# llrtt/G-NeRF

Measured on AMD Instinct MI355X. Metric: rays/sec at 128^2 neural render, 96 depth samples, higher is better.
Workload: dtype f32 (MLP products as compensated f16 hi/lo splits on MFMA, fp32 accumulate; exact-fp32 MFMA when the device-side range check says so)

## Files before the change

### g-nerf_amd/csrc/common.h

```cpp
#pragma once

#include <hip/hip_runtime.h>
#include <hip/hip_fp16.h>
#include <cstdarg>
#include <cstdio>
#include <cstdint>

#include "gnerf_hip.h"

namespace gnerf {

char* error_buffer();

inline int fail(int code, const char* fmt, ...) {
    va_list ap;
    va_start(ap, fmt);
    vsnprintf(error_buffer(), 512, fmt, ap);
    va_end(ap);
    return code;
}

inline int check_launch(const char* what) {
    hipError_t e = hipGetLastError();
    if (e != hipSuccess) return fail(GNERF_E_LAUNCH, "%s: %s", what, hipGetErrorString(e));
    return GNERF_OK;
}

inline hipStream_t as_stream(gnerf_stream_t s) { return reinterpret_cast<hipStream_t>(s); }

struct PerDeviceOnce {
    bool done[64] = {};
    template <class K> int raise_lds(K kernel, const char* what, int bytes = 160 * 1024) {
        int dev = 0;
        if (hipGetDevice(&dev) != hipSuccess || dev < 0 || dev >= 64) dev = -1;
        if (dev >= 0 && done[dev]) return GNERF_OK;
        if (hipFuncSetAttribute(reinterpret_cast<const void*>(kernel), hipFuncAttributeMaxDynamicSharedMemorySize, bytes) != hipSuccess)
            return fail(GNERF_E_LAUNCH, "%s: cannot raise the dynamic LDS limit", what);
        if (dev >= 0) done[dev] = true;
        return GNERF_OK;
    }
};

template <class T> struct Arith { typedef float type; };
template <> struct Arith<double> { typedef double type; };

template <class T> __device__ __forceinline__ typename Arith<T>::type load_as(const T* p, int64_t i) {
    return static_cast<typename Arith<T>::type>(p[i]);
}
template <> __device__ __forceinline__ float load_as<__half>(const __half* p, int64_t i) { return __half2float(p[i]); }

template <class T> __device__ __forceinline__ void store_as(T* p, int64_t i, typename Arith<T>::type v) { p[i] = static_cast<T>(v); }
template <> __device__ __forceinline__ void store_as<__half>(__half* p, int64_t i, float v) { p[i] = __float2half(v); }

constexpr int kNumCU = 256;
constexpr int kNumXCD = 8;

template <class T, int VEC> struct alignas(sizeof(T) * VEC) Pk { T v[VEC]; };
template <class T> __device__ __forceinline__ float round_to(float v) { return v; }
template <> __device__ __forceinline__ float round_to<__half>(float v) { return __half2float(__float2half(v)); }

constexpr int kActLrelu01 = 13;
template <class T, int VEC, int ACT, bool SCALE, bool NOISE, bool NEXT>
__device__ __forceinline__ Pk<T, VEC> modconv_epilogue_vec(const Pk<T, VEC>& in, const float (&sc)[VEC], float nz, bool round_noise, const float (&bv)[VEC],
                                                          const float (&nx)[VEC], float alpha, float gain, float clamp) {
    float t[VEC];
    if constexpr (sizeof(T) == 2 && VEC % 2 == 0 && (SCALE || NOISE)) {
        typedef _Float16 h2 __attribute__((ext_vector_type(2)));
#pragma unroll
        for (int k = 0; k < VEC; k += 2) {
            const h2 xv = {__builtin_bit_cast(_Float16, in.v[k]), __builtin_bit_cast(_Float16, in.v[k + 1])};
            const h2 s2 = {(_Float16)sc[k], (_Float16)sc[k + 1]};
            h2 r;
            if constexpr (NOISE) {
                if (round_noise || SCALE) {
                    const h2 n2 = {(_Float16)nz, (_Float16)nz};
                    r = __builtin_elementwise_fma(xv, s2, n2);
                } else {
                    r = (h2){(_Float16)((float)xv[0] + nz), (_Float16)((float)xv[1] + nz)};
                }
            } else {
                r = xv * s2;
            }
            t[k] = (float)r[0];
            t[k + 1] = (float)r[1];
        }
    } else {
#pragma unroll
        for (int k = 0; k < VEC; k++) {
            float uu = float(load_as<T>(in.v, k));
            if constexpr (SCALE || NOISE) uu = round_to<T>(fmaf(uu, SCALE ? round_to<T>(sc[k]) : 1.f, NOISE ? ((round_noise || SCALE) ? round_to<T>(nz) : nz) : 0.f));
            t[k] = uu;
        }
    }
    Pk<T, VEC> out;
    const bool slope01 = alpha >= 0.f && alpha <= 1.f;
#pragma unroll
    for (int k = 0; k < VEC; k++) {
        const float uu = t[k] + bv[k];
        float r = uu;
        if (ACT == 3) r = slope01 ? fmaxf(uu, uu * alpha) : (uu > 0.f ? uu : uu * alpha);
        if (ACT == kActLrelu01) r = fmaxf(uu, uu * alpha);
        r *= gain;
        if (clamp >= 0.f) r = __builtin_amdgcn_fmed3f(r, -clamp, clamp);
        if constexpr (sizeof(T) == 2 && VEC % 2 == 0) {
            t[k] = r;
        } else {
            if constexpr (NEXT) r = round_to<T>(r) * nx[k];
            store_as<T>(out.v, k, r);
// ... 18 lines not shown
```

### g-nerf_amd/csrc/planes.hip

```cpp

#include "common.h"
#include "raygen.h"

namespace {

using namespace gnerf;

#ifndef GNERF_REPACK_PX
#define GNERF_REPACK_PX 64
#endif
constexpr int CT = 32, PT = GNERF_REPACK_PX;

__device__ __forceinline__ unsigned abs_bits(float v) { return __float_as_uint(v) & 0x7fffffffu; }
__device__ __forceinline__ void publish_absmax(unsigned m, unsigned* out) {
    __shared__ unsigned wave_max[4];
#pragma unroll
    for (int o = 32; o > 0; o >>= 1) m = max(m, (unsigned)__shfl_xor((int)m, o));
    if ((threadIdx.x & 63) == 0) wave_max[threadIdx.x >> 6] = m;
    __syncthreads();
    if (threadIdx.x == 0) {
        const unsigned b = max(max(wave_max[0], wave_max[1]), max(wave_max[2], wave_max[3]));
        if (b > __hip_atomic_load(out, __ATOMIC_RELAXED, __HIP_MEMORY_SCOPE_AGENT)) atomicMax(out, b);
    }
}

template <bool STATS>
__global__ __launch_bounds__(256) void nchw_to_nhwc_kernel(const float* __restrict__ src, float* __restrict__ dst,
                                                           int c, int64_t hw, int tiles_p, int tiles_c, unsigned* absmax) {
    __shared__ float tile[CT][PT + 1];
    int64_t t = blockIdx.x;
    const int tp = int(t % tiles_p); t /= tiles_p;
    const int tc = int(t % tiles_c); t /= tiles_c;
    const int64_t plane = t;
    const int64_t p0 = int64_t(tp) * PT;
    const int c0 = tc * CT;
    const float* s = src + plane * c * hw;
    float* d = dst + plane * hw * c;
    unsigned amax = 0u;
#pragma unroll
    for (int i = 0; i < CT * PT / 256; i++) {
        const int e = threadIdx.x + 256 * i;
        const int ch = e / PT, px = e % PT;
        float v = 0.f;
        if (c0 + ch < c && p0 + px < hw) v = s[int64_t(c0 + ch) * hw + p0 + px];
        tile[ch][px] = v;
        if (STATS) amax = max(amax, abs_bits(v));
    }
    __syncthreads();
#pragma unroll
    for (int i = 0; i < CT * PT / 256; i++) {
        const int e = threadIdx.x + 256 * i;
        const int px = e / CT, ch = e % CT;
        if (c0 + ch < c && p0 + px < hw) d[(p0 + px) * c + c0 + ch] = tile[ch][px];
    }
    if (STATS) publish_absmax(amax, absmax);
}

__global__ __launch_bounds__(256) void absmax_kernel(const float* __restrict__ x, int64_t numel, unsigned* absmax) {
    unsigned amax = 0u;
    const int64_t n4 = numel >> 2;
    const float4* x4 = reinterpret_cast<const float4*>(x);
    const int64_t stride = int64_t(gridDim.x) * 256;
    if (n4 > 0) {
        for (int64_t i = int64_t(blockIdx.x) * 256 + threadIdx.x; i < n4; i += 8 * stride) {
            float4 v[8];
#pragma unroll
            for (int k = 0; k < 8; k++) { const int64_t idx = i + k * stride; v[k] = x4[idx < n4 ? idx : n4 - 1]; }
#pragma unroll
            for (int k = 0; k < 8; k++) amax = max(max(amax, abs_bits(v[k].x)), max(max(abs_bits(v[k].y), abs_bits(v[k].z)), abs_bits(v[k].w)));
        }
    }
    if (blockIdx.x == 0 && threadIdx.x < (numel & 3)) amax = max(amax, abs_bits(x[(n4 << 2) + threadIdx.x]));
    publish_absmax(amax, absmax);
}

struct Up2Taps { float k[4][4]; };

constexpr int kUpCh = 32, kUpRows = 4, kUpCols = 32, kUpInPitch = 4 * 18 + 1, kUpOutPitch = kUpCh + 4;

__global__ __launch_bounds__(256) void upsample2x_add_nhwc_kernel(const float* __restrict__ img, const float* __restrict__ y, Up2Taps K,
                                                                  float* __restrict__ out, int c, int h, int w, unsigned* absmax) {
    __shared__ float in[kUpCh * kUpInPitch];
    __shared__ __align__(16) float ot[kUpRows * kUpCols * kUpOutPitch];
    const int OH = 2 * h, OW = 2 * w;
    const int tiles_x = OW / kUpCols, tiles_y = OH / kUpRows, groups = c / kUpCh;
    int b = blockIdx.x;
    if (gridDim.x % kNumXCD == 0) b = (blockIdx.x % kNumXCD) * (gridDim.x / kNumXCD) + blockIdx.x / kNumXCD;
    const int tx0 = b % tiles_x; b /= tiles_x;
    const int ty0 = b % tiles_y; b /= tiles_y;
    const int cg0 = b % groups;  b /= groups;
    const int n = b;
    const int ox0 = tx0 * kUpCols, oy0 = ty0 * kUpRows, c0 = cg0 * kUpCh;
    const int ix0 = ox0 / 2 - 1, iy0 = oy0 / 2 - 1;
    const float* img_n = img + (int64_t(n) * c + c0) * h * w;
    for (int e = threadIdx.x; e < kUpCh * 4 * 18; e += 256) {
        const int ch = e / 72, r = (e % 72) / 18, cc = e % 18;
        const int iy = iy0 + r, ix = ix0 + cc;
        float v = 0.f;
        if (iy >= 0 && iy < h && ix >= 0 && ix < w) v = img_n[(int64_t(ch) * h + iy) * w + ix];
        in[ch * kUpInPitch + r * 18 + cc] = v;
    }
    __syncthreads();
    {
        const int x4 = threadIdx.x & 7, ty = (threadIdx.x >> 3) & 3, chq = threadIdx.x >> 5;
        const int ry = ty & 1, r = (ty >> 1) + ry;
        const int oy = oy0 + ty;
        float v[4][4];
#pragma unroll
// ... 91 lines not shown
    auto draw = [&](float* __restrict__ out, int64_t numel, const TorchRandDraw& d, uint32_t threads) {
        if (!out || i >= int64_t(threads)) return;
        const int64_t per_thread = (numel - i + int64_t(threads) - 1) / int64_t(threads);
        for (int64_t call = 0; 4 * call < per_thread; call++) {
            const uint64_t c = d.ctr + uint64_t(call);
            uint32_t w[4];
            philox4x32_10_block(uint32_t(c), uint32_t(c >> 32), uint32_t(i), 0u, d.k0, d.k1, w);
#pragma unroll
            for (int k = 0; k < 4; k++) {
                const int64_t li = i + int64_t(threads) * (4 * call + k);
                if (li < numel) {
                    const float u = __fmaf_rn(float(w[k]), 0x1p-32f, 0x1p-32f);
                    out[li] = u == 1.0f ? 0.0f : u;
                }
            }
        }
    };
    draw(out_a, numel_a, da, threads_a);
    draw(out_b, numel_b, db, threads_b);
}

__global__ __launch_bounds__(256) void torch_rand_kernel(float* __restrict__ out, int64_t numel, TorchRandDraw d) {
    const int64_t i = int64_t(blockIdx.x) * 256 + threadIdx.x;
    if (i < numel) out[i] = torch_rand_element(d, uint64_t(i));
}

__global__ __launch_bounds__(256) void to_uint8_nhwc_kernel(const float* __restrict__ img, unsigned char* __restrict__ out, int c, int64_t hw, int64_t total) {
    const int64_t i = int64_t(blockIdx.x) * 256 + threadIdx.x;
    if (i >= total) return;
    const int64_t n = i / hw, p = i - n * hw;
    const float* src = img + n * c * hw + p;
    unsigned char* dst = out + i * c;
    for (int ch = 0; ch < c; ch++) {
        float m = src[int64_t(ch) * hw] * 127.5f;
        asm volatile("" : "+v"(m));
        const float v = m + 128.f;
        dst[ch] = (unsigned char)fminf(fmaxf(v, 0.f), 255.f);
    }
}

}

extern "C" int gnerf_to_uint8_nhwc(const float* img, unsigned char* out, int n, int c, int h, int w, gnerf_stream_t stream) {
    using namespace gnerf;
    if (!img || !out) return fail(GNERF_E_ARG, "to_uint8_nhwc: null pointer");
    if (n < 1 || c < 1 || c > 64 || h < 1 || w < 1) return fail(GNERF_E_ARG, "to_uint8_nhwc: bad shape (1 <= channels <= 64)");
    const int64_t hw = int64_t(h) * w, total = hw * n;
    const int64_t blocks = (total + 255) / 256;
    if (blocks > INT32_MAX) return fail(GNERF_E_ARG, "to_uint8_nhwc: tensor too large");
    hipLaunchKernelGGL(to_uint8_nhwc_kernel, dim3((unsigned)blocks), dim3(256), 0, as_stream(stream), img, out, c, hw, total);
    return check_launch("to_uint8_nhwc");
}

static int planes_to_nhwc_impl(const float* planes_nchw, float* planes_nhwc, int np, int c, int h, int w, float* absmax, bool stats,
                               gnerf_stream_t stream) {
    using namespace gnerf;
    if (!planes_nchw || !planes_nhwc || (stats && !absmax)) return fail(GNERF_E_ARG, "planes_to_nhwc: null pointer");
    if (np < 1 || c < 1 || h < 1 || w < 1) return fail(GNERF_E_ARG, "planes_to_nhwc: empty tensor");
    const int64_t hw = int64_t(h) * w;
    const int tiles_p = int((hw + PT - 1) / PT), tiles_c = (c + CT - 1) / CT;
    const int64_t blocks = int64_t(tiles_p) * tiles_c * np;
    if (blocks > INT32_MAX) return fail(GNERF_E_ARG, "planes_to_nhwc: tensor too large");
    if (stats) {
        if (hipMemsetAsync(absmax, 0, sizeof(float), as_stream(stream)) != hipSuccess) return fail(GNERF_E_LAUNCH, "planes_to_nhwc: memset failed");
        hipLaunchKernelGGL(nchw_to_nhwc_kernel<true>, dim3((unsigned)blocks), dim3(256), 0, as_stream(stream),
                           planes_nchw, planes_nhwc, c, hw, tiles_p, tiles_c, reinterpret_cast<unsigned*>(absmax));
    } else {
        hipLaunchKernelGGL(nchw_to_nhwc_kernel<false>, dim3((unsigned)blocks), dim3(256), 0, as_stream(stream),
                           planes_nchw, planes_nhwc, c, hw, tiles_p, tiles_c, static_cast<unsigned*>(nullptr));
    }
    return check_launch("planes_to_nhwc");
}

extern "C" int gnerf_planes_to_nhwc(const float* planes_nchw, float* planes_nhwc, int np, int c, int h, int w,
                                    gnerf_stream_t stream) {
    return planes_to_nhwc_impl(planes_nchw, planes_nhwc, np, c, h, w, nullptr, false, stream);
}

extern "C" int gnerf_planes_to_nhwc_stats(const float* planes_nchw, float* planes_nhwc, int np, int c, int h, int w,
                                          float* absmax, gnerf_stream_t stream) {
    return planes_to_nhwc_impl(planes_nchw, planes_nhwc, np, c, h, w, absmax, true, stream);
}

extern "C" int gnerf_upsample2x_add_nhwc(const float* img, const float* y, const float* f_host, int flip, float gain, float* out,
                                         int n, int c, int h, int w, float* absmax, gnerf_stream_t stream) {
    using namespace gnerf;
    if (!img || !f_host || !out) return fail(GNERF_E_ARG, "upsample2x_add_nhwc: null pointer");
    if (n < 1 || c < 1 || h < 1 || w < 1) return fail(GNERF_E_ARG, "upsample2x_add_nhwc: empty tensor");
    if (c % kUpCh != 0 || (2 * w) % kUpCols != 0 || (2 * h) % kUpRows != 0) return fail(GNERF_E_UNSUPPORTED, "upsample2x_add_nhwc: needs channels %% 32 == 0, width %% 16 == 0, height %% 2 == 0");
    if ((y && (reinterpret_cast<uintptr_t>(y) & 15)) || (reinterpret_cast<uintptr_t>(out) & 15))
        return fail(GNERF_E_UNSUPPORTED, "upsample2x_add_nhwc: y and out must be 16-byte aligned");
    const int64_t blocks = int64_t(n) * (c / kUpCh) * (2 * h / kUpRows) * (2 * w / kUpCols);
    if (blocks > INT32_MAX || int64_t(n) * c * 4 * h * w > INT32_MAX * int64_t(2)) return fail(GNERF_E_ARG, "upsample2x_add_nhwc: tensor too large");
    Up2Taps K;
    for (int ky = 0; ky < 4; ky++)
        for (int kx = 0; kx < 4; kx++) K.k[ky][kx] = gain * (flip ? f_host[ky * 4 + kx] : f_host[(3 - ky) * 4 + (3 - kx)]);
    if (absmax && hipMemsetAsync(absmax, 0, sizeof(float), as_stream(stream)) != hipSuccess) return fail(GNERF_E_LAUNCH, "upsample2x_add_nhwc: memset failed");
    hipLaunchKernelGGL(upsample2x_add_nhwc_kernel, dim3((unsigned)blocks), dim3(256), 0, as_stream(stream), img, y, K, out, c, h, w,
                       reinterpret_cast<unsigned*>(absmax));
    return check_launch("upsample2x_add_nhwc");
}

extern "C" int gnerf_planes_absmax(const float* planes, int64_t numel, float* absmax, gnerf_stream_t stream) {
    using namespace gnerf;
    if (!planes || !absmax) return fail(GNERF_E_ARG, "planes_absmax: null pointer");
    if (numel < 1) return fail(GNERF_E_ARG, "planes_absmax: empty tensor");
    if (reinterpret_cast<uintptr_t>(planes) & 15) return fail(GNERF_E_ARG, "planes_absmax: planes must be 16-byte aligned");
    if (hipMemsetAsync(absmax, 0, sizeof(float), as_stream(stream)) != hipSuccess) return fail(GNERF_E_LAUNCH, "planes_absmax: memset failed");
    const int64_t n4 = numel / 4, per_trip = int64_t(256) * 8;
    const int64_t trips = (n4 + per_trip * kNumCU * 8 - 1) / (per_trip * kNumCU * 8);
    int64_t blocks = trips > 0 ? (n4 + per_trip * trips - 1) / (per_trip * trips) : 1;
    if (blocks < 1) blocks = 1;
    hipLaunchKernelGGL(absmax_kernel, dim3((unsigned)blocks), dim3(256), 0, as_stream(stream), planes, numel, reinterpret_cast<unsigned*>(absmax));
    return check_launch("planes_absmax");
}

extern "C" int gnerf_planes_from_nhwc(const float* planes_nhwc, float* planes_nchw, int np, int c, int h, int w,
                                      gnerf_stream_t stream) {
    using namespace gnerf;
    if (!planes_nchw || !planes_nhwc) return fail(GNERF_E_ARG, "planes_from_nhwc: null pointer");
    if (np < 1 || c < 1 || h < 1 || w < 1) return fail(GNERF_E_ARG, "planes_from_nhwc: empty tensor");
    const int64_t hw = int64_t(h) * w;
    const int tiles_p = int((hw + PT - 1) / PT), tiles_c = (c + CT - 1) / CT;
    const int64_t blocks = int64_t(tiles_p) * tiles_c * np;
    if (blocks > INT32_MAX) return fail(GNERF_E_ARG, "planes_from_nhwc: tensor too large");
    hipLaunchKernelGGL(nhwc_to_nchw_kernel, dim3((unsigned)blocks), dim3(256), 0, as_stream(stream),
                       planes_nhwc, planes_nchw, c, hw, tiles_p, tiles_c);
    return check_launch("planes_from_nhwc");
}

extern "C" int gnerf_make_rays(const float* cam2world, const float* intrinsics, int n, int res,
                               float* origins, float* dirs, gnerf_stream_t stream) {
    using namespace gnerf;
    if (!cam2world || !intrinsics || !origins || !dirs) return fail(GNERF_E_ARG, "make_rays: null pointer");
// ... 51 lines not shown
```

### g-nerf_amd/csrc/render.hip

```cpp

#include "common.h"
#include "raygen.h"
#include <cstdlib>
#include <cstring>

namespace {

using namespace gnerf;

typedef float v4f __attribute__((ext_vector_type(4)));

constexpr int kHidden = 64;
constexpr int kStagePitch = 36;
constexpr int kRaysPerWave = 16;

struct Params {
    gnerf_render_params p;
    float box_scale;
    float delta;
    float inv_start, inv_end, disp_delta;
    int tiles_c, tiles_f;
    int n_tiles;
    int tiles_per_item, tiles_y;
    int total_rays;
// ... 610 lines not shown
            sq2 = fmaxf(sq2, __shfl_xor(sq2, o)); mx2 = fmaxf(mx2, __shfl_xor(mx2, o));
            mb1 = fmaxf(mb1, __shfl_xor(mb1, o)); mb2 = fmaxf(mb2, __shfl_xor(mb2, o));
        }
        bad = __any(bad);
        if (lane == 0) {
            const float A = *P.absmax;
            const float R1 = sqrtf(sq1), R2 = sqrtf(sq2);
            const float h_hard = l1 * A + mb1 + 1.f;
            const float e_p = 0x1p-22f * R1 * A + 0x1p-25f * (R1 + 5.657f * A);
            const float h = R1 * A + mb1 + 1.f;
            const float e_o = R2 * e_p + 0x1p-22f * R2 * h + 0x1p-25f * (R2 + 8.f * h);
            const bool ok = !bad && A <= kMlpRangeLimit && mx1 <= kMlpRangeLimit && mx2 <= kMlpRangeLimit && h_hard <= kMlpRangeLimit
                            && mb2 <= kMlpRangeLimit && e_o <= kMlpErrLimit;
            const int choice = ok ? 1 : 2;
            reinterpret_cast<int*>(smem)[0] = choice;
            reinterpret_cast<int*>(smem)[1] = (ok && h_hard <= kSoftplusDirectLimit) ? 1 : 0;
            if (blockIdx.x == 0 && p.workspace) static_cast<int*>(p.workspace)[4] = choice;
        }
    }
    __syncthreads();
    const int choice = __builtin_amdgcn_readfirstlane(reinterpret_cast<const int*>(smem)[0]);
    if (softplus_direct) *softplus_direct = __builtin_amdgcn_readfirstlane(reinterpret_cast<const int*>(smem)[1]) != 0;
    __syncthreads();
    return choice;
}

#include "render_shade.inl"
#include "render_pipe.inl"
#include "render_bwd.inl"


int check_common(const gnerf_render_params* p) {
    if (!p) return fail(GNERF_E_ARG, "render: params is null");
    if (!p->planes_nhwc || !p->w1 || !p->b1 || !p->w2 || !p->b2) return fail(GNERF_E_ARG, "render: planes and decoder weights must not be null");
    if (p->n_items < 1 || p->plane_h < 1 || p->plane_w < 1) return fail(GNERF_E_ARG, "render: bad plane shape");
    if (int64_t(p->planes_shared ? 1 : p->n_items) * 3 * p->plane_h * p->plane_w * 32 > INT32_MAX * int64_t(4))
        return fail(GNERF_E_ARG, "render: planes too large");
    if (!(p->box_warp > 0.f)) return fail(GNERF_E_ARG, "render: box_warp must be positive");
    if (p->planes_interleaved != 0 && p->planes_interleaved != 1) return fail(GNERF_E_ARG, "render: planes_interleaved must be 0 or 1");
    return GNERF_OK;
}

void fill_pitches(Params& P) {
    const unsigned W = unsigned(P.p.plane_w), H = unsigned(P.p.plane_h);
    P.tex_pitch = P.p.planes_interleaved ? 384u : 128u;
    P.row_pitch = P.tex_pitch * W;
    P.plane_pitch = P.p.planes_interleaved ? 128u : H * W * 128u;
}

#include "scatter_binned.inl"

}

extern "C" size_t gnerf_render_workspace_bytes(void) { return size_t(kClampItemWord0 + 2 * kClampMaxItems) * 4; }

static int fill_params(const gnerf_render_params* p, Params& P) {
    using namespace gnerf;
    if (int e = check_common(p)) return e;
    const bool own_rays = !p->ray_origins && !p->ray_dirs && p->cam2world && p->intrinsics;
    if (!own_rays && (!p->ray_origins || !p->ray_dirs)) return fail(GNERF_E_ARG, "render: rays must not be null (or both null with cam2world and intrinsics given)");
    if (!own_rays && (p->cam2world || p->intrinsics)) return fail(GNERF_E_ARG, "render: give ray tensors or cam2world / intrinsics, not both");
    if (own_rays && (p->image_width < 1 || int64_t(p->image_width) * p->image_width != p->rays_per_item))
        return fail(GNERF_E_ARG, "render: in-kernel rays need rays_per_item = image_width^2");
    if (p->rng_mode != GNERF_RNG_TENSORS && p->rng_mode != GNERF_RNG_TORCH_PHILOX) return fail(GNERF_E_ARG, "render: rng_mode %d is not one of GNERF_RNG_*", p->rng_mode);
    if (p->rng_mode == GNERF_RNG_TENSORS && !p->noise_coarse) return fail(GNERF_E_ARG, "render: noise_coarse must not be null");
    if (p->rng_mode == GNERF_RNG_TORCH_PHILOX && (p->noise_coarse || p->noise_fine)) return fail(GNERF_E_ARG, "render: rng_mode = GNERF_RNG_TORCH_PHILOX takes no noise tensors");
    const int S = p->depth_resolution, F = p->depth_resolution_importance;
    if (S < 2 || S > GNERF_MAX_SAMPLES) return fail(GNERF_E_ARG, "render: depth_resolution %d outside [2, %d]", S, GNERF_MAX_SAMPLES);
    if (F < 0 || F > GNERF_MAX_SAMPLES) return fail(GNERF_E_ARG, "render: depth_resolution_importance %d outside [0, %d]", F, GNERF_MAX_SAMPLES);
    if (F > 0 && S < 4) return fail(GNERF_E_ARG, "render: importance sampling needs depth_resolution >= 4");
    if (F > 0 && !p->noise_fine && p->rng_mode == GNERF_RNG_TENSORS) return fail(GNERF_E_ARG, "render: noise_fine is null but depth_resolution_importance > 0");
    if (p->sigma_noise_fine && !p->sigma_noise_coarse) return fail(GNERF_E_ARG, "render: sigma_noise_fine without sigma_noise_coarse");
    if (p->sigma_noise_coarse && F > 0 && !p->sigma_noise_fine) return fail(GNERF_E_ARG, "render: sigma_noise_coarse is given but sigma_noise_fine is null with depth_resolution_importance > 0");
    if (p->sigma_noise_coarse && (own_rays || p->rng_mode != GNERF_RNG_TENSORS)) return fail(GNERF_E_UNSUPPORTED, "render: density noise comes with ray and noise tensors (not with in-kernel rays / draws)");
    if (p->rays_per_item < 1) return fail(GNERF_E_ARG, "render: rays_per_item must be positive");
    if ((p->ray_start_per_ray == nullptr) != (p->ray_end_per_ray == nullptr)) return fail(GNERF_E_ARG, "render: per-ray start and end must be given together");
    const int64_t total = int64_t(p->n_items) * p->rays_per_item;
    if (total * (S + F) > INT32_MAX * int64_t(8)) return fail(GNERF_E_ARG, "render: too many samples in one call");

    P.p = *p;
    fill_pitches(P);
    if ((p->planes_shared != 0 && p->planes_shared != 1) || (p->depth_clamp_per_item != 0 && p->depth_clamp_per_item != 1))
        return fail(GNERF_E_ARG, "render: planes_shared and depth_clamp_per_item must be 0 or 1");
    if (p->depth_clamp_per_item && p->n_items > kClampMaxItems) return fail(GNERF_E_ARG, "render: depth_clamp_per_item supports at most %d items", kClampMaxItems);
    P.item_bytes = p->planes_shared ? 0 : int64_t(3) * p->plane_h * p->plane_w * 128;
    if (P.row_pitch >= (1u << 24)) return fail(GNERF_E_UNSUPPORTED, "render: plane rows wider than 2^24 bytes");
    P.box_scale = float(2.0 / double(p->box_warp));
    P.delta = float((double(p->ray_end) - double(p->ray_start)) / double(S - 1));
    P.inv_start = float(1.0 / double(p->ray_start));
    P.inv_end = float(1.0 / double(p->ray_end));
    P.disp_delta = float(1.0 / double(S - 1));
    P.tiles_c = (S + 15) / 16;
    P.tiles_f = (F + 15) / 16;
    P.total_rays = int(total);
    P.split_shift = 0;
    P.pipe_unit = 8;
    P.absmax = nullptr;
    P.draw_c = P.draw_f = TorchRandDraw{};
    P.draw_item_ctr = 0;
    if (p->rng_mode == GNERF_RNG_TORCH_PHILOX) {
        const int64_t units = p->rng_per_item ? int64_t(p->rays_per_item) : total;
        if ((p->rng_per_item != 0 && p->rng_per_item != 1) || p->rng_offset_item_stride % 4 != 0)
            return fail(GNERF_E_ARG, "render: rng_per_item must be 0 or 1 and rng_offset_item_stride a multiple of 4");
        if (!torch_rand_draw(p->rng_seed, p->rng_offset_coarse, p->rng_threads_coarse, units * S, P.draw_c) ||
            (F > 0 && !torch_rand_draw(p->rng_seed, p->rng_offset_fine, p->rng_threads_fine, units * F, P.draw_f)))
            return fail(GNERF_E_UNSUPPORTED, "render: the generator geometry (threads %u / %u, offsets %llu / %llu) is not one the in-kernel draws reproduce",
                        p->rng_threads_coarse, p->rng_threads_fine, (unsigned long long)p->rng_offset_coarse, (unsigned long long)p->rng_offset_fine);
// ... 304 lines not shown
```

### g-nerf_amd/gnerf_hip/__init__.py

```python

import ctypes
import os

import torch

_HERE = os.path.dirname(os.path.abspath(__file__))
LIB_PATH = os.environ.get('GNERF_HIP_LIB') or os.path.join(_HERE, 'libgnerf_hip.so')

_lib = None

F32, F16, F64 = 0, 1, 2
_DTYPE_CODE = {torch.float32: F32, torch.float16: F16, torch.float64: F64}

MAX_SAMPLES = 256
DEBUG_SLOTS = 8
ABI_VERSION = 11
MLP_MODES = {'auto': 0, 'f16x3': 1, 'f32': 2}

_c_p = ctypes.c_void_p
_c_i = ctypes.c_int
_c_i64 = ctypes.c_int64
_c_f = ctypes.c_float


class RenderParams(ctypes.Structure):
    _fields_ = [
        ('planes_nhwc', _c_p), ('n_items', ctypes.c_int32), ('plane_h', ctypes.c_int32), ('plane_w', ctypes.c_int32),
        ('ray_origins', _c_p), ('ray_dirs', _c_p), ('rays_per_item', ctypes.c_int32), ('image_width', ctypes.c_int32),
        ('w1', _c_p), ('b1', _c_p), ('w2', _c_p), ('b2', _c_p),
        ('depth_resolution', ctypes.c_int32), ('depth_resolution_importance', ctypes.c_int32),
        ('ray_start', _c_f), ('ray_end', _c_f),
        ('ray_start_per_ray', _c_p), ('ray_end_per_ray', _c_p),
        ('box_warp', _c_f), ('white_back', ctypes.c_int32), ('disparity_space_sampling', ctypes.c_int32),
        ('noise_coarse', _c_p), ('noise_fine', _c_p),
        ('out_rgb', _c_p), ('out_depth', _c_p), ('out_wsum', _c_p),
        ('workspace', _c_p), ('debug', _c_p),
        ('planes_absmax', _c_p), ('mlp_mode', ctypes.c_int32), ('planes_interleaved', ctypes.c_int32),
        ('planes_shared', ctypes.c_int32), ('depth_clamp_per_item', ctypes.c_int32),
        ('cam2world', _c_p), ('intrinsics', _c_p), ('rng_mode', ctypes.c_int32), ('rng_per_item', ctypes.c_int32),
        ('rng_seed', ctypes.c_uint64), ('rng_offset_coarse', ctypes.c_uint64), ('rng_offset_fine', ctypes.c_uint64),
        ('rng_offset_item_stride', ctypes.c_uint64), ('rng_threads_coarse', ctypes.c_uint32), ('rng_threads_fine', ctypes.c_uint32),
        ('sigma_noise_coarse', _c_p), ('sigma_noise_fine', _c_p),
    ]


class RenderGrads(ctypes.Structure):
    _fields_ = [
        ('grad_rgb', _c_p), ('grad_depth', _c_p), ('grad_wsum', _c_p),
        ('grad_planes_nhwc', _c_p),
        ('grad_w1', _c_p), ('grad_b1', _c_p), ('grad_w2', _c_p), ('grad_b2', _c_p),
        ('scatter_stage', _c_p),
    ]


SIGNATURES = {
    'gnerf_abi_version': (_c_i, []),
    'gnerf_last_error': (ctypes.c_char_p, []),
    'gnerf_build_info': (ctypes.c_char_p, []),
    'gnerf_clock_sample': (_c_i, [_c_p, ctypes.c_double, _c_p]),
    'gnerf_bias_act': (_c_i, [_c_p, _c_p, _c_p, _c_p, _c_p, _c_p, _c_i, _c_i64, _c_i, _c_i64, _c_i, _c_i, _c_f, _c_f, _c_f, _c_p]),
    'gnerf_upfirdn2d': (_c_i, [_c_p, _c_p, _c_p, _c_i, _c_i, _c_i, _c_i, _c_i, ctypes.POINTER(_c_i64), _c_i, _c_i, ctypes.POINTER(_c_i64),
                               _c_i, _c_i, ctypes.POINTER(_c_i64), _c_i, _c_i, _c_i, _c_i, _c_i, _c_i, _c_i, _c_f, _c_p]),
    'gnerf_filtered_lrelu_act': (_c_i, [_c_p, _c_p, _c_i, _c_i, _c_i, _c_i, _c_i, ctypes.POINTER(_c_i64), _c_i, _c_i, _c_i, _c_i,
                                        _c_f, _c_f, _c_f, _c_i, _c_p]),
    'gnerf_filtered_lrelu': (_c_i, [_c_p, _c_p, _c_p, _c_p, _c_p, _c_p, _c_i, _c_i, _c_i, _c_i, _c_i, ctypes.POINTER(_c_i64),
                                    _c_i, _c_i, ctypes.POINTER(_c_i64), _c_i, _c_i, _c_i, _c_i, _c_i, _c_i, _c_i, _c_i,
                                    _c_i, _c_i, _c_i, _c_i, _c_i, _c_f, _c_f, _c_f, _c_i, _c_p]),
    'gnerf_grid_sample_2d': (_c_i, [_c_p, _c_p, _c_p, _c_i, _c_i, _c_i, _c_i, _c_i, ctypes.POINTER(_c_i64), _c_i, _c_i, _c_p]),
    'gnerf_grid_sample_2d_backward': (_c_i, [_c_p, _c_p, _c_p, _c_p, _c_p, _c_i, _c_i, _c_i, _c_i, _c_i, ctypes.POINTER(_c_i64), _c_i, _c_i, _c_p]),
    'gnerf_planes_to_nhwc': (_c_i, [_c_p, _c_p, _c_i, _c_i, _c_i, _c_i, _c_p]),
    'gnerf_planes_to_nhwc_stats': (_c_i, [_c_p, _c_p, _c_i, _c_i, _c_i, _c_i, _c_p, _c_p]),
    'gnerf_planes_absmax': (_c_i, [_c_p, _c_i64, _c_p, _c_p]),
    'gnerf_planes_from_nhwc': (_c_i, [_c_p, _c_p, _c_i, _c_i, _c_i, _c_i, _c_p]),
    'gnerf_make_rays': (_c_i, [_c_p, _c_p, _c_i, _c_i, _c_p, _c_p, _c_p]),
    'gnerf_torch_rand_plan': (_c_i, [_c_i64, _c_i, _c_i, ctypes.POINTER(ctypes.c_uint32), ctypes.POINTER(ctypes.c_uint64)]),
    'gnerf_torch_rand': (_c_i, [_c_p, _c_i64, ctypes.c_uint64, ctypes.c_uint64, ctypes.c_uint32, _c_p]),
    'gnerf_to_uint8_nhwc': (_c_i, [_c_p, _c_p, _c_i, _c_i, _c_i, _c_i, _c_p]),
    'gnerf_render_workspace_bytes': (ctypes.c_size_t, []),
    'gnerf_render_forward': (_c_i, [ctypes.POINTER(RenderParams), _c_p]),
    'gnerf_render_backward': (_c_i, [ctypes.POINTER(RenderParams), ctypes.POINTER(RenderGrads), _c_p]),
    'gnerf_render_backward_stage_bytes': (ctypes.c_size_t, [ctypes.POINTER(RenderParams)]),
    'gnerf_render_backward_exchange_bytes': (ctypes.c_size_t, [ctypes.POINTER(RenderParams)]),
    'gnerf_query_points': (_c_i, [_c_p, _c_i, _c_i, _c_i, _c_p, _c_i, _c_f, _c_p, _c_p, _c_p, _c_p, _c_p, _c_p, _c_i, _c_p]),
    'gnerf_query_points_backward': (_c_i, [_c_p, _c_i, _c_i, _c_i, _c_p, _c_i, _c_f, _c_p, _c_p, _c_p, _c_p, _c_p, _c_p,
                                           _c_p, _c_p, _c_p, _c_p, _c_p, _c_i, _c_p]),
    'gnerf_modulate_weights': (_c_i, [_c_p, _c_p, _c_p, _c_i, _c_p, _c_i, _c_i, _c_i, _c_i, _c_i, _c_i, _c_i, _c_p]),
    'gnerf_normalise_styles': (_c_i, [_c_p, _c_p, _c_i, _c_i, _c_p]),
    'gnerf_scale_channels': (_c_i, [_c_p, _c_p, _c_p, _c_i, _c_i, _c_i, _c_p]),
    'gnerf_modconv_epilogue': (_c_i, [_c_p, _c_p, _c_i, _c_i, _c_i, _c_i, _c_p, _c_p, _c_i, _c_i, _c_p, _c_i, _c_f, _c_f, _c_f, _c_p]),
    'gnerf_conv3x3_epilogue_nhwc': (_c_i, [_c_p, _c_p, _c_p, _c_i, _c_i, _c_i, _c_i, _c_i, _c_p, _c_p, _c_i, _c_p, _c_f, _c_f, _c_f, _c_p, _c_p]),
    'gnerf_conv_transpose3x3_s2_nhwc': (_c_i, [_c_p, _c_p, _c_p, _c_i, _c_i, _c_i, _c_i, _c_i, _c_p]),
    'gnerf_conv3x3_epilogue_torgb_nhwc': (_c_i, [_c_p, _c_p, _c_i, _c_i, _c_i, _c_i, _c_p, _c_p, _c_i, _c_p, _c_f, _c_f, _c_f, _c_p, _c_p, _c_f, _c_p, _c_p]),
    'gnerf_split_f16x3_nhwc': (_c_i, [_c_p, _c_p, _c_p, _c_i, _c_i, _c_i, _c_p, _c_p]),
    'gnerf_make_rays_and_draws': (_c_i, [_c_p, _c_p, _c_i, _c_i, _c_p, _c_p, _c_p, ctypes.c_int64, ctypes.c_uint64, ctypes.c_uint32,
                                         _c_p, ctypes.c_int64, ctypes.c_uint64, ctypes.c_uint32, ctypes.c_uint64, _c_p]),
    'gnerf_conv3x3_f32x3_epilogue_nhwc': (_c_i, [_c_p, _c_p, _c_p, _c_i, _c_i, _c_i, _c_i, _c_i, _c_p, _c_p, _c_p, _c_f, _c_f, _c_f, _c_p, _c_p]),
    'gnerf_conv_transpose3x3_s2_f32x3_nhwc': (_c_i, [_c_p, _c_p, _c_p, _c_i, _c_i, _c_i, _c_i, _c_i, _c_p]),
    'gnerf_upsample2x_add_nhwc': (_c_i, [_c_p, _c_p, ctypes.POINTER(_c_f), _c_i, _c_f, _c_p, _c_i, _c_i, _c_i, _c_i, _c_p, _c_p]),
    'gnerf_scale_channels_nhwc': (_c_i, [_c_p, _c_p, _c_p, _c_i, _c_i, _c_i, _c_i, _c_p]),
    'gnerf_modconv_epilogue_nhwc': (_c_i, [_c_p, _c_p, _c_i, _c_i, _c_i, _c_i, _c_p, _c_p, _c_i, _c_i, _c_p, _c_i, _c_f, _c_f, _c_f, _c_p, _c_p]),
    'gnerf_torgb_nhwc': (_c_i, [_c_p, _c_p, _c_p, _c_p, _c_p, _c_i, _c_i, _c_i, _c_f, _c_p]),
    'gnerf_torgb_nhwc_accumulate': (_c_i, [_c_p, _c_p, _c_p, _c_p, _c_p, _c_i, _c_i, _c_i, _c_f, _c_p]),
    'gnerf_blur4_epilogue_nhwc': (_c_i, [_c_p, _c_p, _c_p, _c_i, _c_i, _c_i, _c_i, _c_i, _c_i, _c_i, _c_i, _c_i, _c_i, _c_f, _c_p, _c_p, _c_i, _c_f, _c_f, _c_f, _c_p, _c_p]),
}


def profiled(name):
    import functools

    def deco(fn):
        @functools.wraps(fn)
        def wrapper(*args, **kwargs):
            if torch.autograd._profiler_enabled():
                with torch.autograd.profiler.record_function(name):
                    return fn(*args, **kwargs)
            return fn(*args, **kwargs)
        return wrapper
    return deco


def load():
    global _lib
    if _lib is not None:
        return _lib
# ... 241 lines not shown
                                           1 if flip_filters else 0, _stream(x))
    if code == E_UNSUPPORTED:
        return none
    _check(code, 'gnerf_filtered_lrelu')
    return y, so, 0


def grid_sample_supported(image, grid):
    return (image.is_cuda and grid.is_cuda and image.ndim == 4 and grid.ndim == 4 and grid.shape[-1] == 2 and grid.shape[0] == image.shape[0]
            and image.dtype in (torch.float32, torch.float16) and image.numel() > 0 and grid.numel() > 0
            and image.stride(2) > 0 and image.stride(3) > 0)


@profiled('gnerf_hip::grid_sample_2d')
def grid_sample_2d(image, grid):
    _require_cuda(image, grid)
    n, c, h, w = image.shape
    ho, wo = grid.shape[1], grid.shape[2]
    g = grid.float().contiguous()
    out = torch.empty([n, c, ho, wo], dtype=image.dtype, device=image.device)
    with _on_device(image.device):
        code = load().gnerf_grid_sample_2d(_ptr(image), _ptr(g), _ptr(out), _DTYPE_CODE[image.dtype], n, c, h, w, _strides(image), ho, wo, _stream(image))
    _check(code, 'gnerf_grid_sample_2d')
    return out


@profiled('gnerf_hip::grid_sample_2d_backward')
def grid_sample_2d_backward(grad_out, image, grid, need_image=True, need_grid=True):
    _require_cuda(grad_out, image, grid)
    n, c, h, w = image.shape
    ho, wo = grid.shape[1], grid.shape[2]
    g = grid.float().contiguous()
    go = grad_out.to(image.dtype).contiguous()
    gi = torch.zeros([n, c, h, w], dtype=torch.float32, device=image.device) if need_image else None
    gg = torch.zeros([n, ho, wo, 2], dtype=torch.float32, device=image.device) if need_grid else None
    with _on_device(image.device):
        code = load().gnerf_grid_sample_2d_backward(_ptr(go), _ptr(image), _ptr(g), _ptr(gi), _ptr(gg), _DTYPE_CODE[image.dtype],
                                                    n, c, h, w, _strides(image), ho, wo, _stream(image))
    _check(code, 'gnerf_grid_sample_2d_backward')
    return (None if gi is None else gi.to(image.dtype)), (None if gg is None else gg.to(grid.dtype))


@profiled('gnerf_hip::planes_to_nhwc')
def planes_to_nhwc(planes, with_absmax=False):
    _require_cuda(planes)
    if planes.dtype != torch.float32:
        raise RuntimeError('planes_to_nhwc: planes must be float32')
    p = planes.reshape(-1, *planes.shape[-3:]).contiguous()
    np_, c, h, w = p.shape
    out = torch.empty([np_, h, w, c], dtype=torch.float32, device=p.device)
    if with_absmax:
        amax = torch.empty([1], dtype=torch.float32, device=p.device)
        with _on_device(p.device):
            code = load().gnerf_planes_to_nhwc_stats(_ptr(p), _ptr(out), np_, c, h, w, _ptr(amax), _stream(p))
        _check(code, 'gnerf_planes_to_nhwc_stats')
        return out, amax
    with _on_device(p.device):
        code = load().gnerf_planes_to_nhwc(_ptr(p), _ptr(out), np_, c, h, w, _stream(p))
    _check(code, 'gnerf_planes_to_nhwc')
    return out


@profiled('gnerf_hip::planes_absmax')
def planes_absmax(planes):
    _require_cuda(planes)
    if planes.dtype != torch.float32 or not planes.is_contiguous() or planes.numel() == 0:
        raise RuntimeError('planes_absmax: expected a non-empty contiguous float32 tensor')
    amax = torch.empty([1], dtype=torch.float32, device=planes.device)
    with _on_device(planes.device):
        code = load().gnerf_planes_absmax(_ptr(planes), planes.numel(), _ptr(amax), _stream(planes))
    _check(code, 'gnerf_planes_absmax')
    return amax


@profiled('gnerf_hip::planes_from_nhwc')
def planes_from_nhwc(planes_nhwc, n_items=None):
    _require_cuda(planes_nhwc)
    if planes_nhwc.dtype != torch.float32 or planes_nhwc.ndim != 4 or not planes_nhwc.is_contiguous():
        raise RuntimeError('planes_from_nhwc: expected a contiguous float32 [NP,H,W,C] tensor')
    np_, h, w, c = planes_nhwc.shape
    out = torch.empty([np_, c, h, w], dtype=torch.float32, device=planes_nhwc.device)
    with _on_device(planes_nhwc.device):
        code = load().gnerf_planes_from_nhwc(_ptr(planes_nhwc), _ptr(out), np_, c, h, w, _stream(planes_nhwc))
    _check(code, 'gnerf_planes_from_nhwc')
    return out if n_items is None else out.view(n_items, np_ // n_items, c, h, w)


@profiled('gnerf_hip::to_uint8_nhwc')
def to_uint8_nhwc(img):
    _require_cuda(img)
    if img.dtype != torch.float32 or img.ndim != 4 or not (1 <= img.shape[1] <= 64):
        raise RuntimeError('to_uint8_nhwc: expected a float32 [N,C,H,W] tensor with 1..64 channels')
    x = img.detach().contiguous()
    n, c, h, w = x.shape
    out = torch.empty([n, h, w, c], dtype=torch.uint8, device=x.device)
    with _on_device(x.device):
        code = load().gnerf_to_uint8_nhwc(_ptr(x), _ptr(out), n, c, h, w, _stream(x))
    _check(code, 'gnerf_to_uint8_nhwc')
    return out


@profiled('gnerf_hip::make_rays')
def make_rays(cam2world, intrinsics, resolution):
    _require_cuda(cam2world, intrinsics)
    c2w = cam2world.to(torch.float32).contiguous()
    k = intrinsics.to(torch.float32).contiguous()
    n = c2w.shape[0]
# ... 828 lines not shown
```

### include/gnerf_hip.h

```cpp
#ifndef GNERF_HIP_H
#define GNERF_HIP_H

#include <stddef.h>
#include <stdint.h>

#ifdef __cplusplus
extern "C" {
#endif

#define GNERF_ABI_VERSION 11

#define GNERF_OK            0
#define GNERF_E_ARG        -1
#define GNERF_E_LAUNCH     -2
#define GNERF_E_UNSUPPORTED -3

#define GNERF_F32 0
#define GNERF_F16 1
#define GNERF_F64 2

typedef void* gnerf_stream_t;

int         gnerf_abi_version(void);
const char* gnerf_last_error(void);
int gnerf_clock_sample(unsigned long long* out, double microseconds, gnerf_stream_t stream);
const char* gnerf_build_info(void);

int gnerf_bias_act(const void* x, const void* b, const void* xref, const void* yref, const void* dy,
                   void* y, int dtype, int64_t numel, int size_b, int64_t step_b,
                   int grad, int act, float alpha, float gain, float clamp, gnerf_stream_t stream);

#define GNERF_W_OIK 0
#define GNERF_W_IOK 1
#define GNERF_W_OKI 2
#define GNERF_W_IKO 3
int gnerf_modulate_weights(const float* weight, const float* styles, void* out, int out_dtype, float* dcoefs,
                           int n, int n_out, int n_in, int kk, int demodulate, int prenorm, int out_layout, gnerf_stream_t stream);
int gnerf_normalise_styles(const float* styles, float* out, int n, int n_in, gnerf_stream_t stream);
int gnerf_scale_channels(const void* x, const float* scale, void* y, int dtype, int rows, int row_len, gnerf_stream_t stream);
int gnerf_modconv_epilogue(const void* x, void* y, int dtype, int rows, int row_len, int channels,
                           const float* scale, const float* noise, int noise_per_item, int round_noise, const void* bias,
                           int act, float alpha, float gain, float clamp, gnerf_stream_t stream);
int gnerf_scale_channels_nhwc(const void* x, const float* scale, void* y, int dtype, int n, int pixels, int channels, gnerf_stream_t stream);
int gnerf_modconv_epilogue_nhwc(const void* x, void* y, int dtype, int n, int pixels, int channels,
                                const float* scale, const float* noise, int noise_per_item, int round_noise, const void* bias,
                                int act, float alpha, float gain, float clamp, const float* next_scale, gnerf_stream_t stream);
int gnerf_blur4_epilogue_nhwc(const void* x, const float* f, void* y, int dtype, int n, int c, int in_h, int in_w, int out_h, int out_w,
                              int padx0, int pady0, int flip, float blur_gain,
                              const float* scale, const void* bias, int act, float alpha, float gain, float clamp, const float* next_scale,
                              gnerf_stream_t stream);
int gnerf_conv3x3_epilogue_nhwc(const void* x, const void* w_packed, void* y, int n, int h, int w, int cin, int cout,
                                const float* scale, const float* noise, int round_noise, const void* bias,
                                float alpha, float gain, float clamp, const float* next_scale, gnerf_stream_t stream);
int gnerf_conv3x3_epilogue_torgb_nhwc(const void* x, const void* w_packed, int n, int h, int w, int cin,
                                      const float* scale, const float* noise, int round_noise, const void* bias,
                                      float alpha, float gain, float clamp,
                                      const void* rgb_w, const float* rgb_bias, float rgb_clamp, float* img, gnerf_stream_t stream);
int gnerf_conv_transpose3x3_s2_nhwc(const void* x, const void* w_phases, void* y, int n, int h, int w, int cin, int cout, gnerf_stream_t stream);
int gnerf_split_f16x3_nhwc(const float* x, const float* scale, void* y, int n, int pixels, int channels, int* overflow, gnerf_stream_t stream);
int gnerf_conv3x3_f32x3_epilogue_nhwc(const void* x3, const void* w3_packed, float* y, int n, int h, int w, int cin3, int cout,
                                      const float* scale, const float* noise, const float* bias,
                                      float alpha, float gain, float clamp, const float* next_scale, gnerf_stream_t stream);
int gnerf_conv_transpose3x3_s2_f32x3_nhwc(const void* x3, const void* w3_phases, float* y, int n, int h, int w, int cin3, int cout, gnerf_stream_t stream);
int gnerf_torgb_nhwc(const void* x, const float* weight, const float* styles, const void* bias, void* y,
                     int n, int pixels, int channels, float clamp, gnerf_stream_t stream);
int gnerf_torgb_nhwc_accumulate(const void* x, const float* weight, const float* styles, const void* bias, float* img,
                                int n, int pixels, int channels, float clamp, gnerf_stream_t stream);

int gnerf_upfirdn2d(const void* x, const float* f, void* y, int dtype,
                    int n, int c, int in_h, int in_w, const int64_t xs[4],
                    int fh, int fw, const int64_t fs[2],
                    int out_h, int out_w, const int64_t ys[4],
                    int upx, int upy, int downx, int downy, int padx0, int pady0,
                    int flip, float gain, gnerf_stream_t stream);

int gnerf_filtered_lrelu_act(void* x, uint8_t* s, int dtype, int n, int c, int h, int w,
                             const int64_t xs[4], int s_h, int s_w, int sx, int sy,
                             float gain, float slope, float clamp, int mode, gnerf_stream_t stream);

int gnerf_filtered_lrelu(const void* x, const float* fu, const float* fd, const void* b, uint8_t* s, void* y,
                         int dtype, int n, int c, int xh, int xw, const int64_t xs[4],
                         int yh, int yw, const int64_t ys[4],
                         int fu_taps, int fu_rank, int fd_taps, int fd_rank,
                         int up, int down, int px0, int py0,
                         int s_h, int s_w, int sx, int sy, int sign_mode,
                         float gain, float slope, float clamp, int flip, gnerf_stream_t stream);

int gnerf_grid_sample_2d(const void* image, const float* grid, void* out, int dtype,
                         int n, int c, int h, int w, const int64_t image_strides[4], int ho, int wo, gnerf_stream_t stream);
int gnerf_grid_sample_2d_backward(const void* grad_out, const void* image, const float* grid, float* grad_image, float* grad_grid,
                                  int dtype, int n, int c, int h, int w, const int64_t image_strides[4], int ho, int wo,
                                  gnerf_stream_t stream);

int gnerf_planes_to_nhwc(const float* planes_nchw, float* planes_nhwc, int np, int c, int h, int w,
                         gnerf_stream_t stream);
int gnerf_planes_to_nhwc_stats(const float* planes_nchw, float* planes_nhwc, int np, int c, int h, int w,
                               float* absmax, gnerf_stream_t stream);
int gnerf_planes_absmax(const float* planes, int64_t numel, float* absmax, gnerf_stream_t stream);
int gnerf_upsample2x_add_nhwc(const float* img, const float* y, const float* f_host, int flip, float gain, float* out,
                              int n, int c, int h, int w, float* absmax, gnerf_stream_t stream);
int gnerf_planes_from_nhwc(const float* planes_nhwc, float* planes_nchw, int np, int c, int h, int w,
                           gnerf_stream_t stream);

int gnerf_to_uint8_nhwc(const float* img, unsigned char* out, int n, int c, int h, int w, gnerf_stream_t stream);

int gnerf_make_rays(const float* cam2world, const float* intrinsics, int n, int res,
                    float* origins, float* dirs, gnerf_stream_t stream);

typedef struct gnerf_render_params {
    const float* planes_nhwc;
    int32_t n_items, plane_h, plane_w;
    const float* ray_origins;
    const float* ray_dirs;
    int32_t rays_per_item;
    int32_t image_width;
    const float* w1; const float* b1; const float* w2; const float* b2;
    int32_t depth_resolution;
    int32_t depth_resolution_importance;
    float   ray_start, ray_end;
    const float* ray_start_per_ray;
    const float* ray_end_per_ray;
    float   box_warp;
    int32_t white_back;
    int32_t disparity_space_sampling;
    const float* noise_coarse;
    const float* noise_fine;
    float* out_rgb;
    float* out_depth;
    float* out_wsum;
    void*  workspace;
    float* debug;
    const float* planes_absmax;
    int32_t mlp_mode;
    int32_t planes_interleaved;
    int32_t planes_shared;
    int32_t depth_clamp_per_item;
    const float* cam2world;
    const float* intrinsics;
    int32_t  rng_mode;
    int32_t  rng_per_item;
    uint64_t rng_seed;
    uint64_t rng_offset_coarse, rng_offset_fine, rng_offset_item_stride;
    uint32_t rng_threads_coarse, rng_threads_fine;
    const float* sigma_noise_coarse;
    const float* sigma_noise_fine;
} gnerf_render_params;

#define GNERF_RNG_TENSORS      0
#define GNERF_RNG_TORCH_PHILOX 1

// ... 59 lines not shown
```

Baseline: 123.2 million.

## Vectorize plane NCHW→NHWC transpose and drop absmax memset via ticketed reduction

Adds a register-only float4 transpose kernel for planes when channels are a multiple of 32 and buffers are 16-byte aligned, replacing the LDS-tiled path. The absmax statistic is now reduced through sharded counters in a persistent workspace, and the last block writes the float result. This removes the separate memset launch and spreads atomic contention. The cost is extra atomics plus reliance on the workspace counters being reset correctly between calls.

After: 126.8 million (median of 6 runs). +2.9%, better.

```diff
diff --git a/g-nerf_amd/csrc/common.h b/g-nerf_amd/csrc/common.h
--- a/g-nerf_amd/csrc/common.h
+++ b/g-nerf_amd/csrc/common.h
@@ -54,6 +54,9 @@
 
 constexpr int kNumCU = 256;
 constexpr int kNumXCD = 8;
+
+constexpr int kStatsWord0 = 8224, kStatsShards = 32, kStatsLineWords = 32;
+constexpr int kWorkspaceWords = kStatsWord0 + (kStatsShards + 1) * kStatsLineWords;
 
 template <class T, int VEC> struct alignas(sizeof(T) * VEC) Pk { T v[VEC]; };
 template <class T> __device__ __forceinline__ float round_to(float v) { return v; }
diff --git a/g-nerf_amd/csrc/planes.hip b/g-nerf_amd/csrc/planes.hip
--- a/g-nerf_amd/csrc/planes.hip
+++ b/g-nerf_amd/csrc/planes.hip
@@ -24,9 +24,34 @@
     }
 }
 
+__device__ __forceinline__ void publish_absmax_ticket(unsigned m, unsigned* ws, float* out) {
+    __shared__ unsigned wave_max[4];
+#pragma unroll
+    for (int o = 32; o > 0; o >>= 1) m = max(m, (unsigned)__shfl_xor((int)m, o));
+    if ((threadIdx.x & 63) == 0) wave_max[threadIdx.x >> 6] = m;
+    __syncthreads();
+    if (threadIdx.x != 0) return;
+    const unsigned b = max(max(wave_max[0], wave_max[1]), max(wave_max[2], wave_max[3]));
+    const unsigned shards = min(gridDim.x, unsigned(kStatsShards));
+    const unsigned s = blockIdx.x % shards, members = (gridDim.x - s + shards - 1) / shards;
+    unsigned* sh = ws + kStatsWord0 + kStatsLineWords * s;
+    unsigned* total = ws + kStatsWord0 + kStatsLineWords * kStatsShards;
+    if (b > __hip_atomic_load(sh, __ATOMIC_RELAXED, __HIP_MEMORY_SCOPE_AGENT)) atomicMax(sh, b);
+    asm volatile("s_waitcnt vmcnt(0)" ::: "memory");
+    if (atomicAdd(sh + 1, 1u) != members - 1) return;
+    const unsigned v = atomicExch(sh, 0u);
+    atomicExch(sh + 1, 0u);
+    if (v > __hip_atomic_load(total, __ATOMIC_RELAXED, __HIP_MEMORY_SCOPE_AGENT)) atomicMax(total, v);
+    asm volatile("s_waitcnt vmcnt(0)" ::: "memory");
+    if (atomicAdd(total + 1, 1u) != shards - 1) return;
+    const unsigned a = atomicExch(total, 0u);
+    atomicExch(total + 1, 0u);
+    *out = __uint_as_float(a);
+}
+
 template <bool STATS>
 __global__ __launch_bounds__(256) void nchw_to_nhwc_kernel(const float* __restrict__ src, float* __restrict__ dst,
-                                                           int c, int64_t hw, int tiles_p, int tiles_c, unsigned* absmax) {
+                                                           int c, int64_t hw, int tiles_p, int tiles_c, unsigned* ws, float* absmax) {
     __shared__ float tile[CT][PT + 1];
     int64_t t = blockIdx.x;
     const int tp = int(t % tiles_p); t /= tiles_p;
@@ -53,7 +78,48 @@
         const int px = e / CT, ch = e % CT;
         if (c0 + ch < c && p0 + px < hw) d[(p0 + px) * c + c0 + ch] = tile[ch][px];
     }
-    if (STATS) publish_absmax(amax, absmax);
+    if (STATS) publish_absmax_ticket(amax, ws, absmax);
+}
+
+constexpr int kV4Trips = 2, kV4Px = 4 * 32 * kV4Trips;
+template <bool STATS>
+__global__ __launch_bounds__(256) void nchw_to_nhwc_v4_kernel(const float* __restrict__ src, float* __restrict__ dst,
+                                                              int c, int64_t hw, int tiles_p, int tiles_c, unsigned* ws, float* absmax) {
+    int64_t t = blockIdx.x;
+    const int tp = int(t % tiles_p); t /= tiles_p;
+    const int tc = int(t % tiles_c); t /= tiles_c;
+    const int64_t plane = t;
+    const int lane = threadIdx.x & 63, wave = threadIdx.x >> 6;
+    const int cg = lane & 7, xg = lane >> 3;
+    const int ch0 = tc * CT + 4 * cg;
+    const float* s = src + (plane * c + ch0) * hw;
+    float* d = dst + plane * hw * c + ch0;
+    float4 v[kV4Trips][4];
+    int64_t px[kV4Trips];
+#pragma unroll
+    for (int j = 0; j < kV4Trips; j++) {
+        px[j] = int64_t(tp) * kV4Px + (j * 4 + wave) * 32 + 4 * xg;
+        const int64_t pl = px[j] < hw ? px[j] : hw - 4;
+#pragma unroll
+        for (int k = 0; k < 4; k++) v[j][k] = *reinterpret_cast<const float4*>(s + k * hw + pl);
+    }
+    unsigned amax = 0u;
+#pragma unroll
+    for (int j = 0; j < kV4Trips; j++) {
+        if (px[j] < hw) {
+            float* o = d + px[j] * c;
+            *reinterpret_cast<float4*>(o)         = make_float4(v[j][0].x, v[j][1].x, v[j][2].x, v[j][3].x);
+            *reinterpret_cast<float4*>(o + c)     = make_float4(v[j][0].y, v[j][1].y, v[j][2].y, v[j][3].y);
+            *reinterpret_cast<float4*>(o + 2 * c) = make_float4(v[j][0].z, v[j][1].z, v[j][2].z, v[j][3].z);
+            *reinterpret_cast<float4*>(o + 3 * c) = make_float4(v[j][0].w, v[j][1].w, v[j][2].w, v[j][3].w);
+        }
+        if (STATS) {
+#pragma unroll
+            for (int k = 0; k < 4; k++)
+                amax = max(max(amax, abs_bits(v[j][k].x)), max(max(abs_bits(v[j][k].y), abs_bits(v[j][k].z)), abs_bits(v[j][k].w)));
+        }
+    }
+    if (STATS) publish_absmax_ticket(amax, ws, absmax);
 }
 
 __global__ __launch_bounds__(256) void absmax_kernel(const float* __restrict__ x, int64_t numel, unsigned* absmax) {
@@ -251,34 +317,34 @@
     return check_launch("to_uint8_nhwc");
 }
 
-static int planes_to_nhwc_impl(const float* planes_nchw, float* planes_nhwc, int np, int c, int h, int w, float* absmax, bool stats,
-                               gnerf_stream_t stream) {
-    using namespace gnerf;
-    if (!planes_nchw || !planes_nhwc || (stats && !absmax)) return fail(GNERF_E_ARG, "planes_to_nhwc: null pointer");
+static int planes_to_nhwc_impl(const float* planes_nchw, float* planes_nhwc, int np, int c, int h, int w, float* absmax, void* workspace,
+                               bool stats, gnerf_stream_t stream) {
+    using namespace gnerf;
+    if (!planes_nchw || !planes_nhwc || (stats && (!absmax || !workspace))) return fail(GNERF_E_ARG, "planes_to_nhwc: null pointer");
     if (np < 1 || c < 1 || h < 1 || w < 1) return fail(GNERF_E_ARG, "planes_to_nhwc: empty tensor");
     const int64_t hw = int64_t(h) * w;
-    const int tiles_p = int((hw + PT - 1) / PT), tiles_c = (c + CT - 1) / CT;
+    const bool v4 = c % CT == 0 && hw % 4 == 0 && !(reinterpret_cast<uintptr_t>(planes_nchw) & 15) && !(reinterpret_cast<uintptr_t>(planes_nhwc) & 15);
+    const int px_tile = v4 ? kV4Px : PT;
+    const int tiles_p = int((hw + px_tile - 1) / px_tile), tiles_c = (c + CT - 1) / CT;
     const int64_t blocks = int64_t(tiles_p) * tiles_c * np;
     if (blocks > INT32_MAX) return fail(GNERF_E_ARG, "planes_to_nhwc: tensor too large");
-    if (stats) {
-        if (hipMemsetAsync(absmax, 0, sizeof(float), as_stream(stream)) != hipSuccess) return fail(GNERF_E_LAUNCH, "planes_to_nhwc: memset failed");
-        hipLaunchKernelGGL(nchw_to_nhwc_kernel<true>, dim3((unsigned)blocks), dim3(256), 0, as_stream(stream),
-                           planes_nchw, planes_nhwc, c, hw, tiles_p, tiles_c, reinterpret_cast<unsigned*>(absmax));
-    } else {
-        hipLaunchKernelGGL(nchw_to_nhwc_kernel<false>, dim3((unsigned)blocks), dim3(256), 0, as_stream(stream),
-                           planes_nchw, planes_nhwc, c, hw, tiles_p, tiles_c, static_cast<unsigned*>(nullptr));
-    }
+    unsigned* ws = static_cast<unsigned*>(workspace);
+    const dim3 grid((unsigned)blocks), block(256);
+    if (v4 && stats) hipLaunchKernelGGL(nchw_to_nhwc_v4_kernel<true>, grid, block, 0, as_stream(stream), planes_nchw, planes_nhwc, c, hw, tiles_p, tiles_c, ws, absmax);
+    else if (v4) hipLaunchKernelGGL(nchw_to_nhwc_v4_kernel<false>, grid, block, 0, as_stream(stream), planes_nchw, planes_nhwc, c, hw, tiles_p, tiles_c, ws, absmax);
+    else if (stats) hipLaunchKernelGGL(nchw_to_nhwc_kernel<true>, grid, block, 0, as_stream(stream), planes_nchw, planes_nhwc, c, hw, tiles_p, tiles_c, ws, absmax);
+    else hipLaunchKernelGGL(nchw_to_nhwc_kernel<false>, grid, block, 0, as_stream(stream), planes_nchw, planes_nhwc, c, hw, tiles_p, tiles_c, ws, absmax);
     return check_launch("planes_to_nhwc");
 }
 
 extern "C" int gnerf_planes_to_nhwc(const float* planes_nchw, float* planes_nhwc, int np, int c, int h, int w,
                                     gnerf_stream_t stream) {
-    return planes_to_nhwc_impl(planes_nchw, planes_nhwc, np, c, h, w, nullptr, false, stream);
+    return planes_to_nhwc_impl(planes_nchw, planes_nhwc, np, c, h, w, nullptr, nullptr, false, stream);
 }
 
 extern "C" int gnerf_planes_to_nhwc_stats(const float* planes_nchw, float* planes_nhwc, int np, int c, int h, int w,
-                                          float* absmax, gnerf_stream_t stream) {
-    return planes_to_nhwc_impl(planes_nchw, planes_nhwc, np, c, h, w, absmax, true, stream);
+                                          float* absmax, void* workspace, gnerf_stream_t stream) {
+    return planes_to_nhwc_impl(planes_nchw, planes_nhwc, np, c, h, w, absmax, workspace, true, stream);
 }
 
 extern "C" int gnerf_upsample2x_add_nhwc(const float* img, const float* y, const float* f_host, int flip, float gain, float* out,
diff --git a/g-nerf_amd/csrc/render.hip b/g-nerf_amd/csrc/render.hip
--- a/g-nerf_amd/csrc/render.hip
+++ b/g-nerf_amd/csrc/render.hip
@@ -686,7 +686,8 @@
 
 }
 
-extern "C" size_t gnerf_render_workspace_bytes(void) { return size_t(kClampItemWord0 + 2 * kClampMaxItems) * 4; }
+static_assert(kClampItemWord0 + 2 * kClampMaxItems <= kStatsWord0, "render words overlap the plane statistics");
+extern "C" size_t gnerf_render_workspace_bytes(void) { return size_t(kWorkspaceWords) * 4; }
 
 static int fill_params(const gnerf_render_params* p, Params& P) {
     using namespace gnerf;
diff --git a/g-nerf_amd/gnerf_hip/__init__.py b/g-nerf_amd/gnerf_hip/__init__.py
--- a/g-nerf_amd/gnerf_hip/__init__.py
+++ b/g-nerf_amd/gnerf_hip/__init__.py
@@ -14,7 +14,7 @@
 
 MAX_SAMPLES = 256
 DEBUG_SLOTS = 8
-ABI_VERSION = 11
+ABI_VERSION = 12
 MLP_MODES = {'auto': 0, 'f16x3': 1, 'f32': 2}
 
 _c_p = ctypes.c_void_p
@@ -69,7 +69,7 @@
     'gnerf_grid_sample_2d': (_c_i, [_c_p, _c_p, _c_p, _c_i, _c_i, _c_i, _c_i, _c_i, ctypes.POINTER(_c_i64), _c_i, _c_i, _c_p]),
     'gnerf_grid_sample_2d_backward': (_c_i, [_c_p, _c_p, _c_p, _c_p, _c_p, _c_i, _c_i, _c_i, _c_i, _c_i, ctypes.POINTER(_c_i64), _c_i, _c_i, _c_p]),
     'gnerf_planes_to_nhwc': (_c_i, [_c_p, _c_p, _c_i, _c_i, _c_i, _c_i, _c_p]),
-    'gnerf_planes_to_nhwc_stats': (_c_i, [_c_p, _c_p, _c_i, _c_i, _c_i, _c_i, _c_p, _c_p]),
+    'gnerf_planes_to_nhwc_stats': (_c_i, [_c_p, _c_p, _c_i, _c_i, _c_i, _c_i, _c_p, _c_p, _c_p]),
     'gnerf_planes_absmax': (_c_i, [_c_p, _c_i64, _c_p, _c_p]),
     'gnerf_planes_from_nhwc': (_c_i, [_c_p, _c_p, _c_i, _c_i, _c_i, _c_i, _c_p]),
     'gnerf_make_rays': (_c_i, [_c_p, _c_p, _c_i, _c_i, _c_p, _c_p, _c_p]),
@@ -417,7 +417,7 @@
     if with_absmax:
         amax = torch.empty([1], dtype=torch.float32, device=p.device)
         with _on_device(p.device):
-            code = load().gnerf_planes_to_nhwc_stats(_ptr(p), _ptr(out), np_, c, h, w, _ptr(amax), _stream(p))
+            code = load().gnerf_planes_to_nhwc_stats(_ptr(p), _ptr(out), np_, c, h, w, _ptr(amax), _workspace(p.device).data_ptr(), _stream(p))
         _check(code, 'gnerf_planes_to_nhwc_stats')
         return out, amax
     with _on_device(p.device):
diff --git a/include/gnerf_hip.h b/include/gnerf_hip.h
--- a/include/gnerf_hip.h
+++ b/include/gnerf_hip.h
@@ -8,7 +8,7 @@
 extern "C" {
 #endif
 
-#define GNERF_ABI_VERSION 11
+#define GNERF_ABI_VERSION 12
 
 #define GNERF_OK            0
 #define GNERF_E_ARG        -1
@@ -95,7 +95,7 @@
 int gnerf_planes_to_nhwc(const float* planes_nchw, float* planes_nhwc, int np, int c, int h, int w,
                          gnerf_stream_t stream);
 int gnerf_planes_to_nhwc_stats(const float* planes_nchw, float* planes_nhwc, int np, int c, int h, int w,
-                               float* absmax, gnerf_stream_t stream);
+                               float* absmax, void* workspace, gnerf_stream_t stream);
 int gnerf_planes_absmax(const float* planes, int64_t numel, float* absmax, gnerf_stream_t stream);
 int gnerf_upsample2x_add_nhwc(const float* img, const float* y, const float* f_host, int flip, float gain, float* out,
                               int n, int c, int h, int w, float* absmax, gnerf_stream_t stream);
```
